# obeychoi0120/wseg

Measured on AMD Instinct MI355X. Metric: training images/sec at B=16x448x448 (contrast_train step), higher is better.
Workload: dtype bf16; 1 GPU; ResNet-38 contrast, synthetic VOC 448x448, B=16/GPU, procedural weights, dropout on, fused HIP loss; global_batch=16, parallelism=dp1, seed=0

## Files before the change

### wseg_amd/csrc/api.hip

```cpp
#include <stdarg.h>
#include <algorithm>
#include "common.h"


static thread_local char g_err[512] = "";
void wseg_set_error(const char* fmt, ...) {
  va_list ap;
  va_start(ap, fmt);
  vsnprintf(g_err, sizeof(g_err), fmt, ap);
  va_end(ap);
}
extern "C" const char* wseg_last_error(void) { return g_err; }
extern "C" int wseg_version(void) { return 101; }
extern "C" size_t wseg_sizeof_conv_desc(void) { return sizeof(wseg_conv_desc); }
extern "C" size_t wseg_sizeof_wgrad_desc(void) { return sizeof(wseg_wgrad_desc); }

namespace {

template <int DT>
__global__ void pack_fwd_kernel(const float* __restrict__ w, void* __restrict__ out, int OC, int T, int IC, int OCp, int ICp, int ic_rot) {
  const size_t total = (size_t)OCp * T * ICp;
  for (size_t i = (size_t)blockIdx.x * blockDim.x + threadIdx.x; i < total; i += (size_t)gridDim.x * blockDim.x) {
    const int ic = (int)(i % ICp);
    const size_t r = i / ICp;
    const int t = (int)(r % T), oc = (int)(r / T);
    const int src = ic + ic_rot >= IC ? ic + ic_rot - IC : ic + ic_rot;
    const float v = (oc < OC && ic < IC) ? w[((size_t)oc * T + t) * IC + src] : 0.f;
    elem<DT>::st(out, i, v);
  }
}
template <int DT>
__global__ void pack_tr_kernel(const float* __restrict__ w, void* __restrict__ out, int OC, int T, int IC, int OCp, int ICp, int ic_rot) {
  __shared__ float tile[32][33];
  const int t = blockIdx.z;
  const int oc0 = blockIdx.y * 32, ic0 = blockIdx.x * 32;
  for (int r = threadIdx.y; r < 32; r += 8) {
    const int oc = oc0 + r, ic = ic0 + threadIdx.x;
    const int src = ic + ic_rot >= IC ? ic + ic_rot - IC : ic + ic_rot;
    tile[r][threadIdx.x] = (oc < OC && ic < IC) ? w[((size_t)oc * T + t) * IC + src] : 0.f;
  }
  __syncthreads();
  for (int r = threadIdx.y; r < 32; r += 8) {
    const int ic = ic0 + r, oc = oc0 + threadIdx.x;
    if (ic < ICp && oc < OCp) elem<DT>::st(out, ((size_t)ic * T + t) * OCp + oc, tile[threadIdx.x][r]);
  }
}

template <int DT>
__global__ void pack_tr_batch_kernel(const float* __restrict__ master, void* __restrict__ out, const long* __restrict__ table, int nlayers) {
  __shared__ float tile[32][33];
  const long bid = blockIdx.x;
  int lo = 0, hi = nlayers - 1;
  while (lo < hi) { const int mid = (lo + hi + 1) >> 1; if (table[mid * 6] <= bid) lo = mid; else hi = mid - 1; }
  const long* e = table + lo * 6;
  const int OC = (int)e[3], T = (int)e[4], IC = (int)e[5];
  const int nti = (IC + 31) / 32, nto = (OC + 31) / 32;
  long r = bid - e[0];
  const int ti = (int)(r % nti); r /= nti;
  const int to = (int)(r % nto); const int t = (int)(r / nto);
  const float* w = master + e[1];
  const int oc0 = to * 32, ic0 = ti * 32;
  for (int rr = threadIdx.y; rr < 32; rr += 8) {
    const int oc = oc0 + rr, ic = ic0 + threadIdx.x;
    tile[rr][threadIdx.x] = (oc < OC && ic < IC) ? w[((size_t)oc * T + t) * IC + ic] : 0.f;
  }
  __syncthreads();
  for (int rr = threadIdx.y; rr < 32; rr += 8) {
    const int ic = ic0 + rr, oc = oc0 + threadIdx.x;
    if (ic < IC && oc < OC) elem<DT>::st(out, (size_t)e[2] + ((size_t)ic * T + t) * OC + oc, tile[threadIdx.x][rr]);
  }
}

__global__ __launch_bounds__(256) void pack_tr_batch_bf16_kernel(const bf16_t* __restrict__ src, bf16_t* __restrict__ out, const long* __restrict__ table, int nlayers) {
  __shared__ bf16_t tile[64][66];
  const long bid = blockIdx.x;
  int lo = 0, hi = nlayers - 1;
  while (lo < hi) { const int mid = (lo + hi + 1) >> 1; if (table[mid * 6] <= bid) lo = mid; else hi = mid - 1; }
  const long* e = table + lo * 6;
  const int OC = (int)e[3], T = (int)e[4], IC = (int)e[5];
  const int nti = (IC + 63) / 64, nto = (OC + 63) / 64;
  long r = bid - e[0];
  const int ti = (int)(r % nti); r /= nti;
  const int to = (int)(r % nto); const int t = (int)(r / nto);
  const bf16_t* w = src + e[1];
  const int oc0 = to * 64, ic0 = ti * 64;
  const int tx = threadIdx.x & 63, ty = threadIdx.x >> 6;
  for (int rr = ty; rr < 64; rr += 4) {
    const int oc = oc0 + rr, ic = ic0 + tx;
    tile[rr][tx] = (oc < OC && ic < IC) ? w[((size_t)oc * T + t) * IC + ic] : (bf16_t)0;
  }
  __syncthreads();
  for (int rr = ty; rr < 64; rr += 4) {
    const int ic = ic0 + rr, oc = oc0 + tx;
    if (ic < IC && oc < OC) out[(size_t)e[2] + ((size_t)ic * T + t) * OC + oc] = tile[tx][rr];
  }
}

__global__ void dropout_scale_kernel(const float* __restrict__ u, float* __restrict__ out, long total, long split_at, float p0, float p1) {
  const long i = (long)blockIdx.x * blockDim.x + threadIdx.x;
  if (i >= total) return;
  const float p = i < split_at ? p0 : p1;
  out[i] = u[i] >= p ? 1.f / (1.f - p) : 0.f;
}

template <int DT, int KC = 0>
__global__ __launch_bounds__(256) void stem_kernel(const float* __restrict__ x, const float* __restrict__ w,
                                                   const float* __restrict__ scale, const float* __restrict__ shift,
                                                   void* raw, void* act, int N, int H, int W) {
  __shared__ __attribute__((aligned(16))) float tile[64 * 68];
  const int tid = threadIdx.x;
  const int nxb = (W + 63) / 64;
  const int bx = blockIdx.x % nxb;
  const int y = (blockIdx.x / nxb) % H;
  const int n = blockIdx.x / (nxb * H);
  const int px = tid & 63, cg = __builtin_amdgcn_readfirstlane(tid >> 6);
  const int xg = bx * 64 + px;
  float in[27];
#pragma unroll
  for (int ic = 0; ic < 3; ++ic)
#pragma unroll
    for (int ky = 0; ky < 3; ++ky) {
      const int iy = y + ky - 1;
#pragma unroll
      for (int kx = 0; kx < 3; ++kx) {
        const int ix = xg + kx - 1;
        in[(ky * 3 + kx) * 3 + ic] = (iy >= 0 && iy < H && ix >= 0 && ix < W) ? x[(((size_t)n * 3 + ic) * H + iy) * W + ix] : 0.f;
      }
    }
  float acc[16];
  if constexpr (KC == 1) {
    typedef float f2_t __attribute__((ext_vector_type(2)));
    const f2_t* wg2 = reinterpret_cast<const f2_t*>(w + cg * 16);
    f2_t a2[8];
#pragma unroll
    for (int o = 0; o < 8; ++o) a2[o] = (f2_t){0.f, 0.f};
#pragma unroll
    for (int ic = 0; ic < 3; ++ic)
#pragma unroll
      for (int t = 0; t < 9; ++t) {
        const f2_t xv = {in[t * 3 + ic], in[t * 3 + ic]};
#pragma unroll
        for (int o = 0; o < 8; ++o) a2[o] = __builtin_elementwise_fma(xv, wg2[(t * 3 + ic) * 32 + o], a2[o]);
      }
#pragma unroll
    for (int o = 0; o < 8; ++o) { acc[2 * o] = a2[o].x; acc[2 * o + 1] = a2[o].y; }
  } else {
  const float* wg = w + (size_t)cg * 16 * 27;
#pragma unroll
  for (int o = 0; o < 16; ++o) {
    float a = 0.f;
#pragma unroll
    for (int ic = 0; ic < 3; ++ic)
#pragma unroll
      for (int t = 0; t < 9; ++t) a = fmaf(in[t * 3 + ic], wg[o * 27 + t * 3 + ic], a);
    acc[o] = a;
  }
  }
  const size_t pix0 = ((size_t)n * H + y) * W + bx * 64;
  const int npx = min(64, W - bx * 64);
  for (int pass = 0; pass < 2; ++pass) {
    void* dst = pass == 0 ? raw : act;
    if (!dst) continue;
    __syncthreads();
#pragma unroll
    for (int o = 0; o < 16; ++o) {
      const int oc = cg * 16 + o;
      float v = acc[o];
      if (pass == 1) v = fmaxf(v * scale[oc] + shift[oc], 0.f);
      tile[px * 68 + oc] = v;
    }
    __syncthreads();
    for (int i = tid; i < 64 * 8; i += 256) {
      const int p = i >> 3, c8 = (i & 7) * 8;
      if (p >= npx) continue;
      float v[8];
      const float4 a0 = *reinterpret_cast<const float4*>(&tile[p * 68 + c8]);
      const float4 a1 = *reinterpret_cast<const float4*>(&tile[p * 68 + c8 + 4]);
      v[0] = a0.x; v[1] = a0.y; v[2] = a0.z; v[3] = a0.w; v[4] = a1.x; v[5] = a1.y; v[6] = a1.z; v[7] = a1.w;
      store8<DT>(dst, (pix0 + p) * 64 + c8, v);
    }
  }
}

}

extern "C" int wseg_pack_weights(const float* master, void* fwd, void* tr, int OC, int T, int IC,
                                 int OCp, int ICp, int ic_rot, int dtype, void* stream) {
  WSEG_CHECK(master && (fwd || tr), "pack_weights: null pointer");
  WSEG_CHECK(OCp >= OC && ICp >= IC && T >= 1 && ic_rot >= 0 && ic_rot < IC, "pack_weights: bad padded shape / rotation");
  hipStream_t s = (hipStream_t)stream;
  if (fwd) {
    const size_t total = (size_t)OCp * T * ICp;
    const int blocks = (int)std::min<size_t>((total + 255) / 256, 4096);
    if (dtype == WSEG_BF16) hipLaunchKernelGGL(pack_fwd_kernel<WSEG_BF16>, dim3(blocks), dim3(256), 0, s, master, fwd, OC, T, IC, OCp, ICp, ic_rot);
    else hipLaunchKernelGGL(pack_fwd_kernel<WSEG_F32>, dim3(blocks), dim3(256), 0, s, master, fwd, OC, T, IC, OCp, ICp, ic_rot);
  }
  if (tr) {
    dim3 grid((ICp + 31) / 32, (OCp + 31) / 32, T);
    if (dtype == WSEG_BF16) hipLaunchKernelGGL(pack_tr_kernel<WSEG_BF16>, grid, dim3(32, 8), 0, s, master, tr, OC, T, IC, OCp, ICp, ic_rot);
    else hipLaunchKernelGGL(pack_tr_kernel<WSEG_F32>, grid, dim3(32, 8), 0, s, master, tr, OC, T, IC, OCp, ICp, ic_rot);
  }
  WSEG_LAUNCH_CHECK();
  return 0;
}

extern "C" int wseg_stem_conv_kc(const float* x, const float* w_kc, const float* scale, const float* shift,
                                 void* raw, void* act, int N, int H, int W, int dtype, void* stream) {
  WSEG_CHECK(x && w_kc && (raw || act), "stem_conv_kc: null pointer");
  WSEG_CHECK(!act || (scale && shift), "stem_conv_kc: act needs scale/shift");
  const long blocks = (long)N * H * ((W + 63) / 64);
  WSEG_CHECK(blocks > 0 && blocks < (1L << 31), "stem_conv_kc: bad shape");
  hipStream_t s = (hipStream_t)stream;
  if (dtype == WSEG_BF16) hipLaunchKernelGGL((stem_kernel<WSEG_BF16, 1>), dim3((unsigned)blocks), dim3(256), 0, s, x, w_kc, scale, shift, raw, act, N, H, W);
  else hipLaunchKernelGGL((stem_kernel<WSEG_F32, 1>), dim3((unsigned)blocks), dim3(256), 0, s, x, w_kc, scale, shift, raw, act, N, H, W);
  WSEG_LAUNCH_CHECK();
  return 0;
}

extern "C" int wseg_stem_conv(const float* x, const float* w, const float* scale, const float* shift,
                              void* raw, void* act, int N, int H, int W, int dtype, void* stream) {
  WSEG_CHECK(x && w && (raw || act), "stem_conv: null pointer");
  WSEG_CHECK(!act || (scale && shift), "stem_conv: act needs scale/shift");
  const long blocks = (long)N * H * ((W + 63) / 64);
  WSEG_CHECK(blocks > 0 && blocks < (1L << 31), "stem_conv: bad shape");
  hipStream_t s = (hipStream_t)stream;
  if (dtype == WSEG_BF16) hipLaunchKernelGGL(stem_kernel<WSEG_BF16>, dim3((unsigned)blocks), dim3(256), 0, s, x, w, scale, shift, raw, act, N, H, W);
  else hipLaunchKernelGGL(stem_kernel<WSEG_F32>, dim3((unsigned)blocks), dim3(256), 0, s, x, w, scale, shift, raw, act, N, H, W);
  WSEG_LAUNCH_CHECK();
  return 0;
}

extern "C" int wseg_pack_transposed_batch(const float* master, void* out, const long* table, int nlayers, long total_tiles, int dtype, void* stream) {
  WSEG_CHECK(master && out && table && nlayers > 0 && total_tiles > 0 && total_tiles < (1L << 31), "pack_transposed_batch: bad arguments");
  hipStream_t s = (hipStream_t)stream;
  if (dtype == WSEG_BF16) hipLaunchKernelGGL(pack_tr_batch_kernel<WSEG_BF16>, dim3((unsigned)total_tiles), dim3(32, 8), 0, s, master, out, table, nlayers);
  else hipLaunchKernelGGL(pack_tr_batch_kernel<WSEG_F32>, dim3((unsigned)total_tiles), dim3(32, 8), 0, s, master, out, table, nlayers);
  WSEG_LAUNCH_CHECK();
  return 0;
}

extern "C" int wseg_dropout_scale(const float* u, float* out, long total, long split_at, float p0, float p1, void* stream) {
  WSEG_CHECK(u && out && total > 0 && p0 >= 0.f && p0 < 1.f && p1 >= 0.f && p1 < 1.f, "dropout_scale: bad arguments");
  hipLaunchKernelGGL(dropout_scale_kernel, dim3((unsigned)((total + 255) / 256)), dim3(256), 0, (hipStream_t)stream, u, out, total, split_at, p0, p1);
  WSEG_LAUNCH_CHECK();
  return 0;
}

extern "C" int wseg_pack_transposed_batch_bf16(const void* mirror, void* out, const long* table, int nlayers, long total_tiles, void* stream) {
  WSEG_CHECK(mirror && out && table && nlayers > 0 && total_tiles > 0 && total_tiles < (1L << 31), "pack_transposed_batch_bf16: bad arguments");
  hipLaunchKernelGGL(pack_tr_batch_bf16_kernel, dim3((unsigned)total_tiles), dim3(256), 0, (hipStream_t)stream, (const bf16_t*)mirror, (bf16_t*)out, table, nlayers);
  WSEG_LAUNCH_CHECK();
  return 0;
}

static __global__ void copy2d_batch_kernel(const uint4* __restrict__ src, uint4* __restrict__ dst, const long* __restrict__ table, int npieces, long total) {
  for (long i = (long)blockIdx.x * blockDim.x + threadIdx.x; i < total; i += (long)gridDim.x * blockDim.x) {
    int lo = 0, hi = npieces - 1;
    while (lo < hi) { const int mid = (lo + hi + 1) >> 1; if (table[mid * 7] <= i) lo = mid; else hi = mid - 1; }
    const long* t = table + lo * 7;
    const long j = i - t[0];
    const long row = j / t[4], c = j - row * t[4];
    dst[t[2] + row * t[6] + c] = src[t[1] + row * t[5] + c];
  }
}
extern "C" int wseg_copy2d_batch(const void* src, void* dst, const long* table, int npieces, long total_chunks, void* stream) {
  WSEG_CHECK(src && dst && table && npieces > 0 && total_chunks > 0 && ((size_t)src & 15) == 0 && ((size_t)dst & 15) == 0, "copy2d_batch: bad arguments");
  const unsigned blocks = (unsigned)std::min<long>((total_chunks + 255) / 256, 8192);
  hipLaunchKernelGGL(copy2d_batch_kernel, dim3(blocks), dim3(256), 0, (hipStream_t)stream, (const uint4*)src, (uint4*)dst, table, npieces, total_chunks);
  WSEG_LAUNCH_CHECK();
  return 0;
}

static __global__ void pack_x3_kernel(const float* src, unsigned char* dst, long nquads) {
  const long idx = (long)blockIdx.x * blockDim.x + threadIdx.x;
  if (idx >= nquads) return;
  const long g = idx >> 3;
  const int q = (int)(idx & 7);
  const float4 v = *reinterpret_cast<const float4*>(src + g * 32 + q * 4);
  const float x[4] = {v.x, v.y, v.z, v.w};
  unsigned short hi[4], lo[4];
#pragma unroll
  for (int e = 0; e < 4; ++e) split_bf16(x[e], hi[e], lo[e]);
  *reinterpret_cast<uint2*>(dst + g * 128 + q * 8) = make_uint2((unsigned)hi[0] | ((unsigned)hi[1] << 16), (unsigned)hi[2] | ((unsigned)hi[3] << 16));
  *reinterpret_cast<uint2*>(dst + g * 128 + 64 + q * 8) = make_uint2((unsigned)lo[0] | ((unsigned)lo[1] << 16), (unsigned)lo[2] | ((unsigned)lo[3] << 16));
}

extern "C" int wseg_pack_x3(const float* src, void* dst, long numel, void* stream) {
  WSEG_CHECK(src && dst && numel > 0 && numel % 32 == 0 && (const void*)src != dst, "pack_x3: numel must be a positive multiple of 32, out of place");
  const long nquads = numel / 4;
  hipLaunchKernelGGL(pack_x3_kernel, dim3((unsigned)((nquads + 255) / 256)), dim3(256), 0, (hipStream_t)stream, src, (unsigned char*)dst, nquads);
  WSEG_LAUNCH_CHECK();
  return 0;
}

static __global__ void split_bf16_kernel(const float* __restrict__ in, bf16_t* __restrict__ hi, bf16_t* __restrict__ lo, long total) {
  const long i = ((long)blockIdx.x * blockDim.x + threadIdx.x) * 8;
  if (i + 7 < total) {
    float v[8];
    load8<WSEG_F32>(in, i, v);
    unsigned h[4], l[4];
#pragma unroll
    for (int j = 0; j < 4; ++j) {
      bf16_t h0, h1, l0, l1;
      split_bf16(v[2 * j], h0, l0);
      split_bf16(v[2 * j + 1], h1, l1);
      h[j] = (unsigned)h0 | ((unsigned)h1 << 16);
      l[j] = (unsigned)l0 | ((unsigned)l1 << 16);
    }
    *reinterpret_cast<uint4*>(hi + i) = make_uint4(h[0], h[1], h[2], h[3]);
    *reinterpret_cast<uint4*>(lo + i) = make_uint4(l[0], l[1], l[2], l[3]);
  } else {
    for (long k = i; k < total; ++k) split_bf16(in[k], hi[k], lo[k]);
  }
}

extern "C" int wseg_split_bf16(const float* in, void* hi, void* lo, long total, void* stream) {
  WSEG_CHECK(in && hi && lo && total > 0, "split_bf16: bad arguments");
  hipLaunchKernelGGL(split_bf16_kernel, dim3((unsigned)((total / 8 + 256) / 256)), dim3(256), 0, (hipStream_t)stream, in, (bf16_t*)hi, (bf16_t*)lo, total);
  WSEG_LAUNCH_CHECK();
  return 0;
}

static __global__ void to_bf16_kernel(const float* __restrict__ in, bf16_t* __restrict__ out, long total) {
  const long i = ((long)blockIdx.x * blockDim.x + threadIdx.x) * 4;
  if (i + 3 < total) {
    const float4 v = *reinterpret_cast<const float4*>(in + i);
    uint2 o;
    o.x = (unsigned)f32_to_bf16(v.x) | ((unsigned)f32_to_bf16(v.y) << 16);
    o.y = (unsigned)f32_to_bf16(v.z) | ((unsigned)f32_to_bf16(v.w) << 16);
    *reinterpret_cast<uint2*>(out + i) = o;
  } else {
    for (long k = i; k < total; ++k) out[k] = f32_to_bf16(in[k]);
  }
}

extern "C" int wseg_to_bf16(const float* in, void* out, long total, void* stream) {
  WSEG_CHECK(in && out && total > 0, "to_bf16: bad arguments");
  hipLaunchKernelGGL(to_bf16_kernel, dim3((unsigned)((total / 4 + 256) / 256)), dim3(256), 0, (hipStream_t)stream, in, (bf16_t*)out, total);
  WSEG_LAUNCH_CHECK();
  return 0;
}
```

### wseg_amd/csrc/conv_wgrad_kernels.h

```cpp
#include <stdlib.h>
#include <algorithm>
#include <type_traits>
#pragma once
#include "common.h"

#ifdef WSEG_PROBES
#define WG_DIAG(a) ((a).diag)
#else
#define WG_DIAG(a) 0
#endif

namespace wseg_wg {
namespace {

template <int OFF>
__device__ __forceinline__ void tr_read(bf16x4& dst, unsigned addr) {
  asm volatile("ds_read_b64_tr_b16 %0, %1 offset:%2" : "=v"(dst) : "v"(addr), "n"(OFF));
}

struct Args {
  wseg_wgrad_desc d;
  int M, taps, nto, nti, ntiles;
  int pix_per_split;
  int nsplit, nwg;
  int simple_adv, q64_1, r64_1, q64_2, r64_2;
  int diag;
};

__device__ __forceinline__ constexpr int swz32(int row) { return (row & 3) | (((row >> 3) & 1) << 2); }

struct WgTile { int tile, split, tap, ky, kx, oc0, ic0, m_begin, m_end; };

template <int BO, int BI>
__device__ __forceinline__ WgTile wg_tile_of(const Args& a, const int bid) {
  WgTile t;
  if ((a.nsplit & 7) == 0) {
    const int xcd = bid & 7, j = bid >> 3, q = a.nsplit >> 3;
    t.tile = j % a.ntiles;
    t.split = xcd * q + j / a.ntiles;
  } else {
    const int l = xcd_remap(bid, a.nwg);
    t.tile = l % a.ntiles;
    t.split = l / a.ntiles;
  }
  t.tap = t.tile % a.taps;
  const int t2 = t.tile / a.taps;
  t.oc0 = t2 / a.nti * BO;
  t.ic0 = t2 % a.nti * BI;
  t.ky = t.tap / a.d.KW;
  t.kx = t.tap - t.ky * a.d.KW;
  t.m_begin = t.split * a.pix_per_split;
  t.m_end = min(a.M, t.m_begin + a.pix_per_split);
  return t;
}

template <int DT, int BO, int BI, int WR, int WC>
__global__ __launch_bounds__(WR * WC * 64, 2) void conv_wgrad_kernel(const Args a) {
  constexpr int NT = WR * WC * 64;
  constexpr int NW = WR * WC;
  constexpr int ES = elem<DT>::size;
  constexpr int CH = 16 / ES;
  constexpr int PK = DT == WSEG_BF16 ? 64 : 32;
  constexpr int ROWB_O = BO * ES, ROWB_I = BI * ES;
  constexpr int TILE_O = PK * ROWB_O, TILE_I = PK * ROWB_I;
  constexpr int STAGE = TILE_O + TILE_I;
  constexpr int MI = BO / WR / 16, NJ = BI / WC / 16;
  constexpr int EPI_ROWS = 64;
  constexpr int EPI_LD = BI + 4;
  constexpr int SMEM = (2 * STAGE > EPI_ROWS * EPI_LD * 4) ? 2 * STAGE : EPI_ROWS * EPI_LD * 4;
  constexpr int PIECES_O = TILE_O / 1024, PIECES_I = TILE_I / 1024;
  static_assert(PIECES_O % NW == 0 && PIECES_I % NW == 0, "pieces must divide over the waves");
  constexpr int PO = PIECES_O / NW, PI = PIECES_I / NW;
  __shared__ __attribute__((aligned(16))) char smem[SMEM];
  const wseg_wgrad_desc& d = a.d;

  const int tid = threadIdx.x, lane = tid & 63;
  const int wid = __builtin_amdgcn_readfirstlane(tid >> 6);
  const WgTile wt = wg_tile_of<BO, BI>(a, blockIdx.x);
  const int tap = wt.tap, ky = wt.ky, kx = wt.kx, oc0 = wt.oc0, ic0 = wt.ic0, m_begin = wt.m_begin, m_end = wt.m_end;
  if (m_begin >= m_end) return;

  const char* zero = reinterpret_cast<const char*>(g_wseg_zero_page);
  const char* X = reinterpret_cast<const char*>(d.x);
  const char* DY = reinterpret_cast<const char*>(d.dy);

  auto logical_chunk = [](int r, int pch) {
    if constexpr (DT == WSEG_BF16) {
      const int s = swz32(r);
      const int blk = pch >> 1;
      return ((((blk & ~7) | ((blk ^ s) & 7))) << 1) | (pch & 1);
    } else {
      const int blk = pch >> 2;
      return (((blk & ~7) | ((blk ^ (r & 7)) & 7)) << 2) | (pch & 3);
    }
  };

  constexpr int CPR_I = ROWB_I / 16, CPR_O = ROWB_O / 16;
  int xr[PI], xlc[PI];
  bool xok[PI];
#pragma unroll
  for (int i = 0; i < PI; ++i) {
    const int ci = (wid * PI + i) * 64 + lane;
    xr[i] = ci / CPR_I;
    xlc[i] = logical_chunk(xr[i], ci % CPR_I);
    xok[i] = (ic0 + xlc[i] * CH) < d.IC;
  }
  int yr[PO], ylc[PO];
  bool yok[PO];
#pragma unroll
  for (int i = 0; i < PO; ++i) {
    const int ci = (wid * PO + i) * 64 + lane;
    yr[i] = ci / CPR_O;
    ylc[i] = logical_chunk(yr[i], ci % CPR_O);
    yok[i] = (oc0 + ylc[i] * CH) < d.OC;
  }

  const int M1 = d.N * d.OH * d.OW;
  int xm[PI], xoy[PI], xox[PI], xbase[PI];
#pragma unroll
  for (int i = 0; i < PI; ++i) {
    xm[i] = m_begin + xr[i];
    const wseg_rowgeo rg = wseg_decode_row(d, min(xm[i], a.M - 1));
    xoy[i] = rg.oy; xox[i] = rg.ox; xbase[i] = (int)rg.in_base;
  }
  auto stage = [&](int buf, int mstep) {
    char* lo = smem + buf * STAGE;
    char* li = lo + TILE_O;
#pragma unroll
    for (int i = 0; i < PO; ++i) {
      const int m = mstep + yr[i];
      const char* po = zero + (lane & 15) * 16;
      if (m < m_end && yok[i]) po = DY + ((size_t)m * d.ld_dy + oc0 + ylc[i] * CH) * ES;
      glds16(po, lo + (wid * PO + i) * 1024);
    }
#pragma unroll
    for (int i = 0; i < PI; ++i) {
      const bool s2 = d.OH2 != 0 && xm[i] >= M1;
      const int OHs = s2 ? d.OH2 : d.OH, OWs = s2 ? d.OW2 : d.OW, IHs = s2 ? d.IH2 : d.IH, IWs = s2 ? d.IW2 : d.IW;
      const char* pi = zero + (lane & 15) * 16;
      if (xm[i] < m_end && xok[i]) {
        const int iy = xoy[i] * d.stride + ky * d.dil - d.pad;
        const int ix = xox[i] * d.stride + kx * d.dil - d.pad;
        if (iy >= 0 && iy < IHs && ix >= 0 && ix < IWs)
          pi = X + ((size_t)(xbase[i] + iy * IWs + ix) * d.ld_x + (size_t)(ic0 + xlc[i] * CH)) * ES;
      }
      glds16(pi, li + (wid * PI + i) * 1024);
      const int mn = xm[i] + PK;
      if (d.OH2 != 0 && xm[i] < M1 && mn >= M1) {
        const wseg_rowgeo rg = wseg_decode_row(d, min(mn, a.M - 1));
        xoy[i] = rg.oy; xox[i] = rg.ox; xbase[i] = (int)rg.in_base;
      } else {
        int ox = xox[i] + PK, oy = xoy[i], bs = xbase[i];
        while (ox >= OWs) { ox -= OWs; ++oy; }
        while (oy >= OHs) { oy -= OHs; bs += IHs * IWs; }
        xox[i] = ox; xoy[i] = oy; xbase[i] = bs;
      }
      xm[i] = mn;
    }
  };

  const int wr = wid / WC, wc = wid % WC;
  const int fcol = lane & 15, fk = lane >> 4;

  f32x4 acc[MI][NJ];
#pragma unroll
  for (int i = 0; i < MI; ++i)
#pragma unroll
    for (int j = 0; j < NJ; ++j) acc[i][j] = (f32x4){0.f, 0.f, 0.f, 0.f};

  const int nk = (m_end - m_begin + PK - 1) / PK;
  stage(0, m_begin);
  __syncthreads();
  int cur = 0;
  for (int kt = 0; kt < nk; ++kt) {
    if (kt + 1 < nk) stage(cur ^ 1, m_begin + (kt + 1) * PK);
    const char* bo = smem + cur * STAGE;
    const char* bi = bo + TILE_O;
    if constexpr (DT == WSEG_BF16) {
      const int q = (lane & 15) >> 2, p = lane & 3;
#pragma unroll
      for (int ks = 0; ks < 2; ++ks) {
        bf16x8 af[MI], bf[NJ];
#pragma unroll
        for (int h = 0; h < 2; ++h) {
          const int row = ks * 32 + fk * 8 + h * 4 + q;
          const int s = swz32(row);
#pragma unroll
          for (int i = 0; i < MI; ++i) {
            const int blk = wr * MI + i;
            const bf16x4 v = __builtin_amdgcn_ds_read_tr16_b64_v4i16(
                (bf16x4 __attribute__((address_space(3)))*)(bo + row * ROWB_O + (((blk & ~7) | ((blk ^ s) & 7)) << 5) + p * 8));
#pragma unroll
            for (int e = 0; e < 4; ++e) af[i][h * 4 + e] = v[e];
          }
#pragma unroll
          for (int j = 0; j < NJ; ++j) {
            const int blk = wc * NJ + j;
            const bf16x4 v = __builtin_amdgcn_ds_read_tr16_b64_v4i16(
                (bf16x4 __attribute__((address_space(3)))*)(bi + row * ROWB_I + (((blk & ~7) | ((blk ^ s) & 7)) << 5) + p * 8));
#pragma unroll
            for (int e = 0; e < 4; ++e) bf[j][h * 4 + e] = v[e];
          }
        }
#pragma unroll
        for (int i = 0; i < MI; ++i)
#pragma unroll
          for (int j = 0; j < NJ; ++j)
            acc[i][j] = __builtin_amdgcn_mfma_f32_16x16x32_bf16(af[i], bf[j], acc[i][j], 0, 0, 0);
      }
    } else if constexpr (DT == WSEG_F32X3) {
      float a8[MI][8], b8[NJ][8];
#pragma unroll
      for (int e = 0; e < 8; ++e) {
        const int row = e * 4 + fk;
        const int s = row & 7;
#pragma unroll
        for (int i = 0; i < MI; ++i) {
          const int blk = wr * MI + i;
          a8[i][e] = *reinterpret_cast<const float*>(bo + row * ROWB_O + (((blk & ~7) | ((blk ^ s) & 7)) << 6) + fcol * 4);
        }
#pragma unroll
        for (int j = 0; j < NJ; ++j) {
          const int blk = wc * NJ + j;
          b8[j][e] = *reinterpret_cast<const float*>(bi + row * ROWB_I + (((blk & ~7) | ((blk ^ s) & 7)) << 6) + fcol * 4);
        }
      }
      bf16x8 ah[MI], al[MI], bh[NJ], bl[NJ];
#pragma unroll
      for (int i = 0; i < MI; ++i) split_bf16x8(a8[i], ah[i], al[i]);
#pragma unroll
      for (int j = 0; j < NJ; ++j) split_bf16x8(b8[j], bh[j], bl[j]);
#pragma unroll
      for (int i = 0; i < MI; ++i)
#pragma unroll
        for (int j = 0; j < NJ; ++j) {
          acc[i][j] = __builtin_amdgcn_mfma_f32_16x16x32_bf16(al[i], bh[j], acc[i][j], 0, 0, 0);
          acc[i][j] = __builtin_amdgcn_mfma_f32_16x16x32_bf16(ah[i], bl[j], acc[i][j], 0, 0, 0);
          acc[i][j] = __builtin_amdgcn_mfma_f32_16x16x32_bf16(ah[i], bh[j], acc[i][j], 0, 0, 0);
        }
    } else {
#pragma unroll
      for (int kk = 0; kk < PK / 4; ++kk) {
        const int row = kk * 4 + fk;
        const int s = row & 7;
        float af[MI], bf[NJ];
#pragma unroll
        for (int i = 0; i < MI; ++i) {
          const int blk = wr * MI + i;
          af[i] = *reinterpret_cast<const float*>(bo + row * ROWB_O + (((blk & ~7) | ((blk ^ s) & 7)) << 6) + fcol * 4);
        }
#pragma unroll
        for (int j = 0; j < NJ; ++j) {
          const int blk = wc * NJ + j;
          bf[j] = *reinterpret_cast<const float*>(bi + row * ROWB_I + (((blk & ~7) | ((blk ^ s) & 7)) << 6) + fcol * 4);
        }
#pragma unroll
        for (int i = 0; i < MI; ++i)
#pragma unroll
          for (int j = 0; j < NJ; ++j)
            acc[i][j] = __builtin_amdgcn_mfma_f32_16x16x4f32(af[i], bf[j], acc[i][j], 0, 0, 0);
      }
    }
    __syncthreads();
    cur ^= 1;
  }

  float* img = reinterpret_cast<float*>(smem);
  const size_t row_stride = (size_t)a.taps * d.IC_dw;
  constexpr int PASSES = BO / EPI_ROWS;
  constexpr int TILES_PER_PASS = EPI_ROWS / 16;
#pragma unroll 1
  for (int ps = 0; ps < PASSES; ++ps) {
#pragma unroll
    for (int i = 0; i < MI; ++i) {
      const int t = wr * MI + i;
      if (t / TILES_PER_PASS == ps) {
        const int row = (t % TILES_PER_PASS) * 16 + fk * 4;
#pragma unroll
        for (int j = 0; j < NJ; ++j) {
          const int col = (wc * NJ + j) * 16 + fcol;
#pragma unroll
          for (int e = 0; e < 4; ++e) img[(row + e) * EPI_LD + col] = acc[i][j][e];
        }
      }
    }
    __syncthreads();
#pragma unroll 1
    for (int idx = tid; idx < EPI_ROWS * BI; idx += NT) {
      const int row = idx / BI, col = idx - row * BI;
      const int oc = oc0 + ps * EPI_ROWS + row, ic = ic0 + col;
      if (oc < d.OC_dw && ic < d.IC_dw) {
        int icw = ic + d.dw_rot;
        icw = icw >= d.IC_dw ? icw - d.IC_dw : icw;
        atomicAdd(&d.dw[(size_t)oc * row_stride + (size_t)tap * d.IC_dw + icw], img[row * EPI_LD + col]);
      }
    }
    __syncthreads();
  }
}

struct StageBase {
  static constexpr int PK = 64, HALF = 16384;
  const Args& a;
  const wseg_wgrad_desc& d;
  const WgTile& t;
  char* const smem;
  const int tid, wid;
  const char* zsrc;
  int lc[2];
  const char* ybase[2];
  size_t ystep;

  __device__ __forceinline__ StageBase(const Args& a_, const WgTile& t_, char* smem_, int tid_, int wid_)
      : a(a_), d(a_.d), t(t_), smem(smem_), tid(tid_), wid(wid_) {
    zsrc = reinterpret_cast<const char*>(g_wseg_zero_page) + (tid & 15) * 16;
    const int pch = tid & 15;
#pragma unroll
    for (int k = 0; k < 2; ++k) {
      lc[k] = (((pch >> 1) ^ swz32(row(k))) << 1) | (pch & 1);
      ybase[k] = reinterpret_cast<const char*>(d.dy) + ((size_t)(t.m_begin + row(k)) * d.ld_dy + t.oc0 + lc[k] * 8) * 2;
    }
    ystep = (size_t)PK * d.ld_dy * 2;
  }
  __device__ __forceinline__ int row(int k) const { return (tid >> 4) + 32 * k; }
  __device__ __forceinline__ char* dst(int buf, int which) const { return smem + (which * 2 + buf) * HALF + wid * 1024; }
};

struct StageGeneral : StageBase {
  bool yok[2][2], xok[2][2];
  int my[2];
  int xm[2], xoy[2], xox[2], xbase[2];
  const char* xrow[2];
  int M1;

  __device__ __forceinline__ StageGeneral(const Args& a_, const WgTile& t_, char* smem_, int tid_, int wid_) : StageBase(a_, t_, smem_, tid_, wid_) {
    M1 = d.N * d.OH * d.OW;
#pragma unroll
    for (int k = 0; k < 2; ++k) {
      my[k] = xm[k] = t.m_begin + row(k);
      const wseg_rowgeo rg = wseg_decode_row(d, min(xm[k], a.M - 1));
      xoy[k] = rg.oy; xox[k] = rg.ox; xbase[k] = (int)rg.in_base;
#pragma unroll
      for (int h = 0; h < 2; ++h) {
        yok[k][h] = t.oc0 + 128 * h + lc[k] * 8 < d.OC;
        xok[k][h] = t.ic0 + 128 * h + lc[k] * 8 < d.IC;
      }
    }
  }
  __device__ __forceinline__ int ntiles() const { return (t.m_end - t.m_begin + PK - 1) / PK; }

  __device__ __forceinline__ void prepare_x() {
#pragma unroll
    for (int k = 0; k < 2; ++k) {
      const bool s2 = d.OH2 != 0 && xm[k] >= M1;
      const int OHs = s2 ? d.OH2 : d.OH, OWs = s2 ? d.OW2 : d.OW, IHs = s2 ? d.IH2 : d.IH, IWs = s2 ? d.IW2 : d.IW;
      const int mn = xm[k] + PK;
      xrow[k] = nullptr;
      if (xm[k] < t.m_end) {
        const int iy = xoy[k] * d.stride + t.ky * d.dil - d.pad;
        const int ix = xox[k] * d.stride + t.kx * d.dil - d.pad;
        if (iy >= 0 && iy < IHs && ix >= 0 && ix < IWs)
          xrow[k] = reinterpret_cast<const char*>(d.x) + ((size_t)(xbase[k] + iy * IWs + ix) * d.ld_x + t.ic0 + lc[k] * 8) * 2;
      }
      if (d.OH2 != 0 && xm[k] < M1 && mn >= M1) {
        const wseg_rowgeo rg = wseg_decode_row(d, min(mn, a.M - 1));
        xoy[k] = rg.oy; xox[k] = rg.ox; xbase[k] = (int)rg.in_base;
      } else if (a.simple_adv) {
        int ox = xox[k] + (s2 ? a.r64_2 : a.r64_1), oy = xoy[k] + (s2 ? a.q64_2 : a.q64_1), bs = xbase[k];
        const bool cx = ox >= OWs;
        ox = cx ? ox - OWs : ox; oy = cx ? oy + 1 : oy;
        const bool cy = oy >= OHs;
        oy = cy ? oy - OHs : oy; bs = cy ? bs + IHs * IWs : bs;
        xox[k] = ox; xoy[k] = oy; xbase[k] = bs;
      } else {
        int ox = xox[k] + PK, oy = xoy[k], bs = xbase[k];
        while (ox >= OWs) { ox -= OWs; ++oy; }
        while (oy >= OHs) { oy -= OHs; bs += IHs * IWs; }
        xox[k] = ox; xoy[k] = oy; xbase[k] = bs;
      }
      xm[k] = mn;
    }
  }
  __device__ __forceinline__ void issue_x(int h, int buf) {
    char* to = dst(buf, 2 + h);
#pragma unroll
    for (int k = 0; k < 2; ++k) {
      const char* p = (xrow[k] && xok[k][h]) ? xrow[k] + h * 256 : zsrc;
      glds16(p, to + k * 8192);
    }
  }
  __device__ __forceinline__ void issue_y(int h, int buf) {
    char* to = dst(buf, h);
#pragma unroll
    for (int k = 0; k < 2; ++k) {
      const char* p = (my[k] < t.m_end && yok[k][h] && WG_DIAG(a) != 5) ? ybase[k] + h * 256 : zsrc;
      glds16(p, to + k * 8192);
    }
    if (h == 1) {
#pragma unroll
      for (int k = 0; k < 2; ++k) { ybase[k] += ystep; my[k] += PK; }
    }
  }
};

struct StageUnit : StageBase {
  int dy, dx;
  const char* xptr[2];
  size_t xstep;
  long xcross;
  int b_begin, nA, nB;
  int ty_idx = 0, tx_idx = 0;
  int y_m, x_m;
  int y_lim, x_lim;
  bool x_s2;
  int xoy[2], xox[2];
  int rry[2][2], rrx[2][2];
  bool xin[2] = {false, false};

  __device__ __forceinline__ StageUnit(const Args& a_, const WgTile& t_, char* smem_, int tid_, int wid_) : StageBase(a_, t_, smem_, tid_, wid_) {
    const int M1 = d.N * d.OH * d.OW;
    dy = t.ky * d.dil - d.pad; dx = t.kx * d.dil - d.pad;
    const bool s2 = d.OH2 != 0 && t.m_begin >= M1;
    const long shift = (long)dy * (s2 ? d.IW2 : d.IW) + dx;
#pragma unroll
    for (int k = 0; k < 2; ++k) {
      const wseg_rowgeo rg = wseg_decode_row(d, min(t.m_begin + row(k), a.M - 1));
      xoy[k] = rg.oy; xox[k] = rg.ox;
      xptr[k] = reinterpret_cast<const char*>(d.x) + (((long)(t.m_begin + row(k)) + shift) * d.ld_x + t.ic0 + lc[k] * 8) * 2;
#pragma unroll
      for (int h = 0; h < 2; ++h) {
        rry[k][h] = t.oc0 + 128 * h + lc[k] * 8 < d.OC ? row(k) : 0x40000000;
        rrx[k][h] = t.ic0 + 128 * h + lc[k] * 8 < d.IC ? row(k) : 0x40000000;
      }
    }
    xstep = (size_t)PK * d.ld_x * 2;
    xcross = (long)dy * (d.IW2 - d.IW) * d.ld_x * 2;
    const int seg_end = d.OH2 != 0 ? M1 : a.M;
    const int a_end = min(t.m_end, seg_end);
    b_begin = max(t.m_begin, seg_end);
    nA = t.m_begin < a_end ? (a_end - t.m_begin + PK - 1) / PK : 0;
    nB = t.m_end > b_begin ? (t.m_end - b_begin + PK - 1) / PK : 0;
    y_m = x_m = t.m_begin;
    y_lim = x_lim = nA > 0 ? a_end : t.m_end;
    x_s2 = nA == 0 && d.OH2 != 0;
  }
  __device__ __forceinline__ int ntiles() const { return nA + nB; }

  __device__ __forceinline__ void prepare_x() {
    if (tx_idx == nA && nA > 0 && nB > 0) {
      const long jump = (long)(b_begin - x_m) * d.ld_x * 2 + xcross;
#pragma unroll
      for (int k = 0; k < 2; ++k) {
        xptr[k] += jump;
        const wseg_rowgeo rg = wseg_decode_row(d, min(b_begin + row(k), a.M - 1));
        xoy[k] = rg.oy; xox[k] = rg.ox;
      }
      x_m = b_begin; x_lim = t.m_end; x_s2 = true;
    }
    const int OHs = x_s2 ? d.OH2 : d.OH, OWs = x_s2 ? d.OW2 : d.OW;
    const int r64 = x_s2 ? a.r64_2 : a.r64_1, q64 = x_s2 ? a.q64_2 : a.q64_1;
#pragma unroll
    for (int k = 0; k < 2; ++k) {
      xin[k] = (unsigned)(xoy[k] + dy) < (unsigned)OHs && (unsigned)(xox[k] + dx) < (unsigned)OWs;
      int ox = xox[k] + r64, oy = xoy[k] + q64;
      const bool cx = ox >= OWs;
      ox = cx ? ox - OWs : ox; oy = cx ? oy + 1 : oy;
      oy = oy >= OHs ? oy - OHs : oy;
      xox[k] = ox; xoy[k] = oy;
    }
  }
  __device__ __forceinline__ void issue_x(int h, int buf) {
    char* to = dst(buf, 2 + h);
    const int rem = WG_DIAG(a) >= 4 ? 0 : x_lim - x_m;
#pragma unroll
    for (int k = 0; k < 2; ++k) {
      const char* p = (xin[k] && rrx[k][h] < rem) ? xptr[k] + h * 256 : zsrc;
      glds16(p, to + k * 8192);
    }
    if (h == 1) {
#pragma unroll
      for (int k = 0; k < 2; ++k) xptr[k] += xstep;
      x_m += PK; ++tx_idx;
    }
  }
  __device__ __forceinline__ void issue_y(int h, int buf) {
    if (h == 0 && ty_idx == nA && nA > 0 && nB > 0) {
      const long jump = (long)(b_begin - y_m) * d.ld_dy * 2;
#pragma unroll
      for (int k = 0; k < 2; ++k) ybase[k] += jump;
      y_m = b_begin; y_lim = t.m_end;
    }
    char* to = dst(buf, h);
    const int rem = WG_DIAG(a) == 5 ? 0 : y_lim - y_m;
#pragma unroll
    for (int k = 0; k < 2; ++k) {
      const char* p = rry[k][h] < rem ? ybase[k] + h * 256 : zsrc;
      glds16(p, to + k * 8192);
    }
    if (h == 1) {
#pragma unroll
      for (int k = 0; k < 2; ++k) ybase[k] += ystep;
      y_m += PK; ++ty_idx;
    }
  }
};

template <int UNIT>
__device__ __forceinline__ void conv_wgrad_pipe_tile(const Args& a, char* smem, const int bid) {
  constexpr int BO = 256, BI = 256;
  constexpr int HALF = 16384, ROWB = 256;
  const wseg_wgrad_desc& d = a.d;
  const int tid = threadIdx.x, lane = tid & 63;
  const int wid = __builtin_amdgcn_readfirstlane(tid >> 6);
  const WgTile wt = wg_tile_of<BO, BI>(a, bid);
  if (wt.m_begin >= wt.m_end) return;
  std::conditional_t<UNIT != 0, StageUnit, StageGeneral> st(a, wt, smem, tid, wid);

  const int wr = wid >> 2, wc = wid & 3;
  const int fcol = lane & 15, fk = lane >> 4;
  const int q = (lane & 15) >> 2, p = lane & 3;
  const unsigned lds0 = (unsigned)(size_t)(__attribute__((address_space(3))) char*)smem;

  f32x4 acc[8][4];
#pragma unroll
  for (int i = 0; i < 8; ++i)
#pragma unroll
    for (int j = 0; j < 4; ++j) acc[i][j] = (f32x4){0.f, 0.f, 0.f, 0.f};

  const int nt = st.ntiles();
  st.issue_y(0, 0); st.issue_y(1, 0);
  st.prepare_x(); st.issue_x(0, 0); st.issue_x(1, 0);
  if (nt > 1) { st.prepare_x(); st.issue_x(0, 1); st.issue_x(1, 1); asm volatile("s_waitcnt vmcnt(4)" ::: "memory"); }
  else asm volatile("s_waitcnt vmcnt(0)" ::: "memory");
  asm volatile("s_barrier" ::: "memory");

  bf16x4 va[2][2][4], vb0[2][2][2], vb1[2][2][2];
  bf16x8 af[2][4], b0[2][2], b1[2][2];
#define PACK_A()                                                                                                \
  _Pragma("unroll") for (int ks = 0; ks < 2; ++ks) _Pragma("unroll") for (int i = 0; i < 4; ++i)               \
    af[ks][i] = __builtin_shufflevector(va[ks][0][i], va[ks][1][i], 0, 1, 2, 3, 4, 5, 6, 7);
#define PACK_B(BF, VB)                                                                                          \
  _Pragma("unroll") for (int ks = 0; ks < 2; ++ks) _Pragma("unroll") for (int j = 0; j < 2; ++j)               \
    BF[ks][j] = __builtin_shufflevector(VB[ks][0][j], VB[ks][1][j], 0, 1, 2, 3, 4, 5, 6, 7);
#define WAIT_LDS() do { asm volatile("s_waitcnt lgkmcnt(0)" ::: "memory"); __builtin_amdgcn_sched_barrier(0); } while (0)
#define MFMA_Q(HA, HB, BF)                                                                                      \
  do {                                                                                                          \
    __builtin_amdgcn_s_setprio(1);                                                                              \
    _Pragma("unroll") for (int ks = 0; ks < 2; ++ks) _Pragma("unroll") for (int i = 0; i < 4; ++i)             \
      _Pragma("unroll") for (int j = 0; j < 2; ++j)                                                            \
        acc[(HA) * 4 + i][(HB) * 2 + j] =                                                                       \
            __builtin_amdgcn_mfma_f32_16x16x32_bf16(af[ks][i], BF[ks][j], acc[(HA) * 4 + i][(HB) * 2 + j], 0, 0, 0); \
    __builtin_amdgcn_s_setprio(0);                                                                              \
  } while (0)

  {
    unsigned LTA[8], LTB[4];
    {
      const unsigned s_ = swz32(fk * 8 + q);
      const unsigned rowterm = lds0 + (unsigned)(fk * 8 + q) * ROWB + (unsigned)p * 8;
#pragma unroll
      for (int t = 0; t < 8; ++t) LTA[t] = rowterm + (((unsigned)t ^ s_) << 5) + (unsigned)(wr * 2) * HALF;
#pragma unroll
      for (int t = 0; t < 4; ++t) LTB[t] = rowterm + (((unsigned)((wc & 1) * 4 + t) ^ s_) << 5) + (unsigned)((2 + (wc >> 1)) * 2) * HALF;
    }
    auto ktile = [&](auto BC, int u) {
      constexpr int b = decltype(BC)::value;
      constexpr int BO = b * HALF;
#pragma unroll
      for (int i = 0; i < 4; ++i) {
        tr_read<BO + 0>(va[0][0][i], LTA[i]); tr_read<BO + 1024>(va[0][1][i], LTA[i]);
        tr_read<BO + 8192>(va[1][0][i], LTA[i]); tr_read<BO + 9216>(va[1][1][i], LTA[i]);
      }
#pragma unroll
      for (int j = 0; j < 2; ++j) {
        tr_read<BO + 0>(vb0[0][0][j], LTB[j]); tr_read<BO + 1024>(vb0[0][1][j], LTB[j]);
        tr_read<BO + 8192>(vb0[1][0][j], LTB[j]); tr_read<BO + 9216>(vb0[1][1][j], LTB[j]);
        tr_read<BO + 0>(vb1[0][0][j], LTB[2 + j]); tr_read<BO + 1024>(vb1[0][1][j], LTB[2 + j]);
        tr_read<BO + 8192>(vb1[1][0][j], LTB[2 + j]); tr_read<BO + 9216>(vb1[1][1][j], LTB[2 + j]);
      }
      if (u + 1 < nt && WG_DIAG(a) != 6) { st.issue_y(0, b ^ 1); st.issue_y(1, b ^ 1); }
      WAIT_LDS();
      PACK_A() PACK_B(b0, vb0) PACK_B(b1, vb1)
      MFMA_Q(0, 0, b0);
      MFMA_Q(0, 1, b1);
      asm volatile("s_barrier" ::: "memory");
#pragma unroll
      for (int i = 0; i < 4; ++i) {
        tr_read<BO + 0>(va[0][0][i], LTA[4 + i]); tr_read<BO + 1024>(va[0][1][i], LTA[4 + i]);
        tr_read<BO + 8192>(va[1][0][i], LTA[4 + i]); tr_read<BO + 9216>(va[1][1][i], LTA[4 + i]);
      }
      if (u + 2 < nt) { if (WG_DIAG(a) != 6) { st.prepare_x(); st.issue_x(0, b); st.issue_x(1, b); } asm volatile("s_waitcnt vmcnt(4)" ::: "memory"); }
      else asm volatile("s_waitcnt vmcnt(0)" ::: "memory");
      WAIT_LDS();
      PACK_A()
      MFMA_Q(1, 1, b1);
      MFMA_Q(1, 0, b0);
      asm volatile("s_barrier" ::: "memory");
    };
    int u = 0;
    for (; u + 1 < nt; u += 2) {
      ktile(std::integral_constant<int, 0>{}, u);
      ktile(std::integral_constant<int, 1>{}, u + 1);
    }
    if (u < nt) ktile(std::integral_constant<int, 0>{}, u);
  }
#undef PACK_A
#undef PACK_B
#undef WAIT_LDS
#undef MFMA_Q
  __syncthreads();

  constexpr int WLD = 64 + 4;
  float* wimg = reinterpret_cast<float*>(smem) + wid * (16 * WLD);
  const size_t row_stride = (size_t)a.taps * d.IC_dw;
  const int ic = wt.ic0 + wc * 64 + lane;
  const bool ic_ok = ic < d.IC_dw;
#pragma unroll
  for (int i = 0; i < 8; ++i) {
#pragma unroll
    for (int j = 0; j < 4; ++j)
#pragma unroll
      for (int e = 0; e < 4; ++e) wimg[(fk * 4 + e) * WLD + j * 16 + fcol] = acc[i][j][e];
    asm volatile("s_waitcnt lgkmcnt(0)" ::: "memory");
    const int oc_base = wt.oc0 + wr * 128 + i * 16;
#pragma unroll
    for (int r = 0; r < 16; ++r) {
      const int oc = oc_base + r;
      if (ic_ok && oc < d.OC_dw) atomicAdd(&d.dw[(size_t)oc * row_stride + (size_t)wt.tap * d.IC_dw + ic], wimg[r * WLD + lane]);
    }
    asm volatile("s_waitcnt lgkmcnt(0)" ::: "memory");
  }
}

template <int UNIT>
__global__ __launch_bounds__(512, 2) void conv_wgrad_pipe_kernel(const Args a) {
  __shared__ __attribute__((aligned(16))) char smem[2 * 4 * 16384];
  conv_wgrad_pipe_tile<UNIT>(a, smem, blockIdx.x);
}

struct Plan { Args a; bool pipe; bool unit; };
static int wgrad_plan(const wseg_wgrad_desc* d, Plan& pl) {
  Args& a = pl.a;
  WSEG_CHECK(d && d->x && d->dy && d->dw, "conv_wgrad: null pointer");
  WSEG_CHECK(d->dtype == WSEG_F32 || d->dtype == WSEG_BF16 || d->dtype == WSEG_F32X3, "conv_wgrad: bad dtype");
  WSEG_CHECK(d->IC % 8 == 0 && d->OC % 8 == 0 && d->ld_x % 8 == 0 && d->ld_dy % 8 == 0,
             "conv_wgrad: IC/OC/ld must be multiples of 8 (IC=%d OC=%d ld_x=%d ld_dy=%d)", d->IC, d->OC, d->ld_x, d->ld_dy);
  WSEG_CHECK(d->ld_x >= d->IC && d->ld_dy >= d->OC, "conv_wgrad: leading dims too small");
  WSEG_CHECK(d->IC_dw > 0 && d->IC_dw <= d->IC && d->OC_dw > 0 && d->OC_dw <= d->OC, "conv_wgrad: bad dw extents");
  WSEG_CHECK(d->dw_rot >= 0 && d->dw_rot < d->IC_dw, "conv_wgrad: dw_rot=%d must lie in [0, IC_dw)", d->dw_rot);
  WSEG_CHECK(d->N > 0 && d->OH > 0 && d->OW > 0 && d->IH > 0 && d->IW > 0 && d->stride >= 1 && d->dil >= 1, "conv_wgrad: bad shape");
  const long M = (long)d->N * d->OH * d->OW + (long)d->N * d->OH2 * d->OW2;
  WSEG_CHECK(d->OH2 >= 0 && (d->OH2 == 0 || (d->OW2 > 0 && d->IH2 > 0 && d->IW2 > 0)), "conv_wgrad: bad second segment");
  WSEG_CHECK(M < (1L << 31), "conv_wgrad: too many pixels");
  const bool big = d->dtype == WSEG_BF16 && d->OC >= 256 && d->IC >= 256 && d->tile_hint != 128 &&
                   (M >= 16384 || d->tile_hint == 256);
  const int BO = big ? 256 : 128, BI = BO;
  a.d = *d;
  a.M = (int)M;
  a.taps = d->KH * d->KW;
  a.nto = (d->OC + BO - 1) / BO;
  a.nti = (d->IC + BI - 1) / BI;
  a.ntiles = a.nto * a.nti * a.taps;
  const int pk = d->dtype == WSEG_BF16 ? 64 : 32;
  int split = d->split_k;
  if (split <= 0) {
    const long slots = big ? 256 : 512;
    const double epi = big ? 28.0 : 10.0;
    const int max_split = (int)std::max(1L, std::min(64L, M / (pk * 8)));
    double best = 1e30;
    split = 1;
    for (int sp = 1; sp <= max_split; ++sp) {
      const long blocks = (long)a.ntiles * sp;
      const long rounds = (blocks + slots - 1) / slots;
      const double steps = (double)((M + sp - 1) / sp + pk - 1) / pk;
      const double cost = rounds * (steps + epi) * (1.0 + 0.002 * sp);
      if (cost < best) { best = cost; split = sp; }
    }
  }
  long pps = (M + split - 1) / split;
  pps = (pps + pk - 1) / pk * pk;
  a.pix_per_split = (int)pps;
  split = (int)((M + pps - 1) / pps);
  a.nsplit = split;
  a.nwg = a.ntiles * split;
  a.q64_1 = 64 / d->OW; a.r64_1 = 64 % d->OW;
  a.q64_2 = d->OH2 ? 64 / d->OW2 : 0; a.r64_2 = d->OH2 ? 64 % d->OW2 : 0;
  a.simple_adv = (a.q64_1 + 1 <= d->OH) && (d->OH2 == 0 || a.q64_2 + 1 <= d->OH2);
#ifdef WSEG_PROBES
  static const int diag = getenv("WSEG_WGRAD_DIAG") ? atoi(getenv("WSEG_WGRAD_DIAG")) : 0;
  a.diag = diag;
#else
  a.diag = 0;
#endif
  pl.unit = a.simple_adv && d->stride == 1 && d->IH == d->OH && d->IW == d->OW && (d->OH2 == 0 || (d->IH2 == d->OH2 && d->IW2 == d->OW2));
  pl.pipe = big;
  WSEG_CHECK(d->dw_rot == 0 || !pl.pipe, "conv_wgrad: dw_rot is supported by the 128-tile kernel only");
  return 0;
}
static void wgrad_plan_report(const Plan& pl, wseg_launch_plan* out) {
  const int t = pl.pipe ? 256 : 128;
  *out = wseg_launch_plan{pl.pipe ? WSEG_WGRAD_256x256 : WSEG_WGRAD_128x128, t, t, pl.a.nwg, 0, 0, pl.a.nsplit, pl.pipe && pl.unit};
}
}
}
```

Before: 475.4 images/sec.

## Pipeline bf16 wgrad LDS reads with inline transposed loads and vectorize weight pack

The bf16 weight-gradient main loop is rewritten with precomputed LDS base addresses, inline-asm ds_read_b64_tr_b16 with immediate offsets, explicit lgkmcnt waits, and a publish step that combines the vmcnt wait with s_barrier. The second k-slice reads are issued early so they overlap with the first slice's MFMAs. Separately, the bf16 transposed weight pack gains a 16-byte vectorized path that uses a swizzled shared tile when pointers and dims are aligned. The aim is less address arithmetic, less LDS latency stall and fewer narrow memory ops, at the cost of hand-managed waits that could be fragile.

Measured after the change: 477.5 images/sec (median of 6 runs). No clear change (+0.5%).

```diff
diff --git a/wseg_amd/csrc/api.hip b/wseg_amd/csrc/api.hip
--- a/wseg_amd/csrc/api.hip
+++ b/wseg_amd/csrc/api.hip
@@ -71,8 +71,8 @@
   }
 }
 
-__global__ __launch_bounds__(256) void pack_tr_batch_bf16_kernel(const bf16_t* __restrict__ src, bf16_t* __restrict__ out, const long* __restrict__ table, int nlayers) {
-  __shared__ bf16_t tile[64][66];
+__global__ __launch_bounds__(256) void pack_tr_batch_bf16_kernel(const bf16_t* __restrict__ src, bf16_t* __restrict__ out, const long* __restrict__ table, int nlayers, int aligned16) {
+  __shared__ __attribute__((aligned(16))) bf16_t tile[64][66];
   const long bid = blockIdx.x;
   int lo = 0, hi = nlayers - 1;
   while (lo < hi) { const int mid = (lo + hi + 1) >> 1; if (table[mid * 6] <= bid) lo = mid; else hi = mid - 1; }
@@ -84,6 +84,35 @@
   const int to = (int)(r % nto); const int t = (int)(r / nto);
   const bf16_t* w = src + e[1];
   const int oc0 = to * 64, ic0 = ti * 64;
+  if (aligned16 && ((IC | OC | e[1] | e[2]) & 7) == 0) {
+    unsigned* t32 = reinterpret_cast<unsigned*>(&tile[0][0]);
+    const int c = threadIdx.x & 7;
+#pragma unroll
+    for (int h = 0; h < 2; ++h) {
+      const int row = (threadIdx.x >> 3) + h * 32;
+      const int oc = oc0 + row, ic = ic0 + c * 8;
+      uint4 v = make_uint4(0u, 0u, 0u, 0u);
+      if (oc < OC && ic < IC) v = *reinterpret_cast<const uint4*>(w + ((size_t)oc * T + t) * IC + ic);
+      *reinterpret_cast<uint4*>(t32 + row * 32 + ((c ^ ((row >> 3) & 7)) << 2)) = v;
+    }
+    __syncthreads();
+    const int p = threadIdx.x >> 3;
+    unsigned wd[8];
+#pragma unroll
+    for (int k = 0; k < 8; ++k) wd[k] = t32[(c * 8 + k) * 32 + ((((p >> 2) ^ c) & 7) << 2) + (p & 3)];
+    uint4 lo4, hi4;
+    lo4.x = (wd[0] & 0xffffu) | (wd[1] << 16); hi4.x = (wd[0] >> 16) | (wd[1] & 0xffff0000u);
+    lo4.y = (wd[2] & 0xffffu) | (wd[3] << 16); hi4.y = (wd[2] >> 16) | (wd[3] & 0xffff0000u);
+    lo4.z = (wd[4] & 0xffffu) | (wd[5] << 16); hi4.z = (wd[4] >> 16) | (wd[5] & 0xffff0000u);
+    lo4.w = (wd[6] & 0xffffu) | (wd[7] << 16); hi4.w = (wd[6] >> 16) | (wd[7] & 0xffff0000u);
+    const int ic = ic0 + 2 * p, oc = oc0 + c * 8;
+    if (ic < IC && oc < OC) {
+      bf16_t* o = out + (size_t)e[2] + ((size_t)ic * T + t) * OC + oc;
+      *reinterpret_cast<uint4*>(o) = lo4;
+      *reinterpret_cast<uint4*>(o + (size_t)T * OC) = hi4;
+    }
+    return;
+  }
   const int tx = threadIdx.x & 63, ty = threadIdx.x >> 6;
   for (int rr = ty; rr < 64; rr += 4) {
     const int oc = oc0 + rr, ic = ic0 + tx;
@@ -248,7 +277,8 @@
 
 extern "C" int wseg_pack_transposed_batch_bf16(const void* mirror, void* out, const long* table, int nlayers, long total_tiles, void* stream) {
   WSEG_CHECK(mirror && out && table && nlayers > 0 && total_tiles > 0 && total_tiles < (1L << 31), "pack_transposed_batch_bf16: bad arguments");
-  hipLaunchKernelGGL(pack_tr_batch_bf16_kernel, dim3((unsigned)total_tiles), dim3(256), 0, (hipStream_t)stream, (const bf16_t*)mirror, (bf16_t*)out, table, nlayers);
+  const int aligned16 = (((size_t)mirror | (size_t)out) & 15) == 0;
+  hipLaunchKernelGGL(pack_tr_batch_bf16_kernel, dim3((unsigned)total_tiles), dim3(256), 0, (hipStream_t)stream, (const bf16_t*)mirror, (bf16_t*)out, table, nlayers, aligned16);
   WSEG_LAUNCH_CHECK();
   return 0;
 }
diff --git a/wseg_amd/csrc/conv_wgrad_kernels.h b/wseg_amd/csrc/conv_wgrad_kernels.h
--- a/wseg_amd/csrc/conv_wgrad_kernels.h
+++ b/wseg_amd/csrc/conv_wgrad_kernels.h
@@ -61,13 +61,14 @@
   constexpr int ES = elem<DT>::size;
   constexpr int CH = 16 / ES;
   constexpr int PK = DT == WSEG_BF16 ? 64 : 32;
+  constexpr int NBUF = 2;
   constexpr int ROWB_O = BO * ES, ROWB_I = BI * ES;
   constexpr int TILE_O = PK * ROWB_O, TILE_I = PK * ROWB_I;
   constexpr int STAGE = TILE_O + TILE_I;
   constexpr int MI = BO / WR / 16, NJ = BI / WC / 16;
   constexpr int EPI_ROWS = 64;
   constexpr int EPI_LD = BI + 4;
-  constexpr int SMEM = (2 * STAGE > EPI_ROWS * EPI_LD * 4) ? 2 * STAGE : EPI_ROWS * EPI_LD * 4;
+  constexpr int SMEM = (NBUF * STAGE > EPI_ROWS * EPI_LD * 4) ? NBUF * STAGE : EPI_ROWS * EPI_LD * 4;
   constexpr int PIECES_O = TILE_O / 1024, PIECES_I = TILE_I / 1024;
   static_assert(PIECES_O % NW == 0 && PIECES_I % NW == 0, "pieces must divide over the waves");
   constexpr int PO = PIECES_O / NW, PI = PIECES_I / NW;
@@ -169,6 +170,66 @@
     for (int j = 0; j < NJ; ++j) acc[i][j] = (f32x4){0.f, 0.f, 0.f, 0.f};
 
   const int nk = (m_end - m_begin + PK - 1) / PK;
+  if constexpr (DT == WSEG_BF16) {
+    static_assert(BO <= 128 && BI <= 128, "one 8-block swizzle group per operand row");
+    static_assert((NBUF - 1) * STAGE + TILE_O + (PK - 32 + 4) * (ROWB_O > ROWB_I ? ROWB_O : ROWB_I) < 65536, "offsets of the transposed reads");
+    const int q = (lane & 15) >> 2, p = lane & 3;
+    const unsigned lds0 = (unsigned)(size_t)(__attribute__((address_space(3))) char*)smem;
+    const unsigned s_ = swz32(fk * 8 + q);
+    unsigned LA[MI], LB[NJ];
+#pragma unroll
+    for (int i = 0; i < MI; ++i) LA[i] = lds0 + (unsigned)(fk * 8 + q) * ROWB_O + (unsigned)p * 8 + ((((unsigned)(wr * MI + i)) ^ s_) << 5);
+#pragma unroll
+    for (int j = 0; j < NJ; ++j) LB[j] = lds0 + (unsigned)(fk * 8 + q) * ROWB_I + (unsigned)p * 8 + ((((unsigned)(wc * NJ + j)) ^ s_) << 5);
+#define WAIT_LDS() do { asm volatile("s_waitcnt lgkmcnt(0)" ::: "memory"); __builtin_amdgcn_sched_barrier(0); } while (0)
+    constexpr int AHEAD = NBUF - 1, RQ = PO + PI, KS = PK / 32;
+    auto publish = [&](int left) {
+      __builtin_amdgcn_sched_barrier(0);
+      if (AHEAD > 2 && left >= 2) asm volatile("s_waitcnt vmcnt(%0)\n\ts_barrier" ::"n"(2 * RQ) : "memory");
+      else if (AHEAD > 1 && left == 1) asm volatile("s_waitcnt vmcnt(%0)\n\ts_barrier" ::"n"(RQ) : "memory");
+      else asm volatile("s_waitcnt vmcnt(0)\n\ts_barrier" ::: "memory");
+      __builtin_amdgcn_sched_barrier(0);
+    };
+#pragma unroll
+    for (int s = 0; s < AHEAD; ++s)
+      if (s < nk) stage(s, m_begin + s * PK);
+    publish(min(AHEAD, nk) - 1);
+    int cur = 0;
+    for (int kt = 0; kt < nk; ++kt) {
+      if (kt + AHEAD < nk) stage(cur == 0 ? NBUF - 1 : cur - 1, m_begin + (kt + AHEAD) * PK);
+      __builtin_amdgcn_sched_barrier(0);
+      const unsigned cb = (unsigned)cur * STAGE;
+      bf16x4 va[2][2][MI], vb[2][2][NJ];
+      bf16x8 af[MI], bf[NJ];
+#pragma unroll
+      for (int i = 0; i < MI; ++i) { tr_read<0>(va[0][0][i], LA[i] + cb); tr_read<4 * ROWB_O>(va[0][1][i], LA[i] + cb); }
+#pragma unroll
+      for (int j = 0; j < NJ; ++j) { tr_read<TILE_O>(vb[0][0][j], LB[j] + cb); tr_read<TILE_O + 4 * ROWB_I>(vb[0][1][j], LB[j] + cb); }
+      WAIT_LDS();
+      if constexpr (KS == 2) {
+#pragma unroll
+        for (int i = 0; i < MI; ++i) { tr_read<32 * ROWB_O>(va[1][0][i], LA[i] + cb); tr_read<36 * ROWB_O>(va[1][1][i], LA[i] + cb); }
+#pragma unroll
+        for (int j = 0; j < NJ; ++j) { tr_read<TILE_O + 32 * ROWB_I>(vb[1][0][j], LB[j] + cb); tr_read<TILE_O + 36 * ROWB_I>(vb[1][1][j], LB[j] + cb); }
+      }
+#pragma unroll
+      for (int ks = 0; ks < KS; ++ks) {
+        if (ks == 1) WAIT_LDS();
+#pragma unroll
+        for (int i = 0; i < MI; ++i) af[i] = __builtin_shufflevector(va[ks][0][i], va[ks][1][i], 0, 1, 2, 3, 4, 5, 6, 7);
+#pragma unroll
+        for (int j = 0; j < NJ; ++j) bf[j] = __builtin_shufflevector(vb[ks][0][j], vb[ks][1][j], 0, 1, 2, 3, 4, 5, 6, 7);
+#pragma unroll
+        for (int i = 0; i < MI; ++i)
+#pragma unroll
+          for (int j = 0; j < NJ; ++j)
+            acc[i][j] = __builtin_amdgcn_mfma_f32_16x16x32_bf16(af[i], bf[j], acc[i][j], 0, 0, 0);
+      }
+      publish(min(AHEAD - 1, nk - 2 - kt));
+      cur = cur == NBUF - 1 ? 0 : cur + 1;
+    }
+#undef WAIT_LDS
+  } else {
   stage(0, m_begin);
   __syncthreads();
   int cur = 0;
@@ -176,39 +237,7 @@
     if (kt + 1 < nk) stage(cur ^ 1, m_begin + (kt + 1) * PK);
     const char* bo = smem + cur * STAGE;
     const char* bi = bo + TILE_O;
-    if constexpr (DT == WSEG_BF16) {
-      const int q = (lane & 15) >> 2, p = lane & 3;
-#pragma unroll
-      for (int ks = 0; ks < 2; ++ks) {
-        bf16x8 af[MI], bf[NJ];
-#pragma unroll
-        for (int h = 0; h < 2; ++h) {
-          const int row = ks * 32 + fk * 8 + h * 4 + q;
-          const int s = swz32(row);
-#pragma unroll
-          for (int i = 0; i < MI; ++i) {
-            const int blk = wr * MI + i;
-            const bf16x4 v = __builtin_amdgcn_ds_read_tr16_b64_v4i16(
-                (bf16x4 __attribute__((address_space(3)))*)(bo + row * ROWB_O + (((blk & ~7) | ((blk ^ s) & 7)) << 5) + p * 8));
-#pragma unroll
-            for (int e = 0; e < 4; ++e) af[i][h * 4 + e] = v[e];
-          }
-#pragma unroll
-          for (int j = 0; j < NJ; ++j) {
-            const int blk = wc * NJ + j;
-            const bf16x4 v = __builtin_amdgcn_ds_read_tr16_b64_v4i16(
-                (bf16x4 __attribute__((address_space(3)))*)(bi + row * ROWB_I + (((blk & ~7) | ((blk ^ s) & 7)) << 5) + p * 8));
-#pragma unroll
-            for (int e = 0; e < 4; ++e) bf[j][h * 4 + e] = v[e];
-          }
-        }
-#pragma unroll
-        for (int i = 0; i < MI; ++i)
-#pragma unroll
-          for (int j = 0; j < NJ; ++j)
-            acc[i][j] = __builtin_amdgcn_mfma_f32_16x16x32_bf16(af[i], bf[j], acc[i][j], 0, 0, 0);
-      }
-    } else if constexpr (DT == WSEG_F32X3) {
+    if constexpr (DT == WSEG_F32X3) {
       float a8[MI][8], b8[NJ][8];
 #pragma unroll
       for (int e = 0; e < 8; ++e) {
@@ -263,6 +292,7 @@
     }
     __syncthreads();
     cur ^= 1;
+  }
   }
 
   float* img = reinterpret_cast<float*>(smem);
```
